# rbrito/deprecated-lame-mirror

Measured on AMD Instinct MI355X. Metric: encoded audio seconds/sec (x real-time) at 44.1kHz stereo CBR128, higher is better.
Workload: dtype f32

## Files before the change

deprecated-lame-mirror_amd/csrc/lh_analysis.hip:

```cpp
#include <stdint.h>
#include <math.h>

#ifdef LH_EMU
#include "hipemu.h"
#define LH_CONST static const
#else
#include <hip/hip_runtime.h>
#define LH_CONST __device__ static const
#endif

#if defined(LH_APROF) && !defined(LH_EMU)
__shared__ unsigned long long *lh_ap_base;
#define LH_PT(var) unsigned long long var = clock64()
#define LH_PA(idx, var) do { if (c.lane == 0) atomicAdd(&lh_ap_base[LH_NPROF * c.wave + 20 + (idx)], clock64() - var); } while (0)
#define LH_PC(idx) do { } while (0)
#endif
#define LH_CUSTOM_LDS "lh_lds_analysis.h"
#define LH_CUSTOM_SMP
#define LH_FZ_X(i) ((((i) >> 4) & 2) | (((i) >> 3) & 24) | (((i) >> 5) & 4))
#define LH_FZ(i) ((i) ^ LH_FZ_X(i))
#define LH_STAGE_IDX(i) LH_FZ(i)
#include "lh_static_tables.h"
#include "lh_dev_common.h"
#if !defined(LH_EMU)
#define LH_KRESTRICT __restrict__
#else
#define LH_KRESTRICT
#endif

#define LH_SPAN (lh_lds.work)
LH_DEVFN float
lh_smp(const LhCtx & c, int ch, int i)
{
    return LH_SPAN[ch * LH_BLKSIZE + LH_FZ(i)];
}

#include "lh_dev_psy_core.h"

struct LhGranuleAt {
    int     live;
    int     gr;
    long long at;
    long long frame_base;
};

LH_DEVFN LhGranuleAt
lh_granule_at(const LhStreamDesc & d, int g)
{
    LhGranuleAt o;
    int const nf = d.frame_end - d.frame_begin;
    int const fr = g / LH_NGR;
    o.live = g < LH_NGR * nf;
    o.gr = g - fr * LH_NGR;
    o.at = d.out_index + d.mid_rel + fr;
    o.frame_base = (long long) (576 * LH_NGR) * (d.frame_begin + fr) - LH_MF_START;
    return o;
}

LH_DEVFN LhStreamDesc
lh_desc_uniform(const LhStreamDesc * descs, int sidx)
{
    LhStreamDesc d = descs[sidx];
    d.pcm_l = lh_uni_ll(d.pcm_l);
    d.pcm_r = lh_uni_ll(d.pcm_r);
    d.pcm_base = lh_uni_ll(d.pcm_base);
    d.nsamples = lh_uni_ll(d.nsamples);
    d.out_index = lh_uni_ll(d.out_index);
    d.mid_rel = lh_uni_i(d.mid_rel);
    d.frame_begin = lh_uni_i(d.frame_begin);
    d.frame_end = lh_uni_i(d.frame_end);
    return d;
}

#ifdef LH_LSF
#define lh_attack_kernel lh_attack_kernel_lsf
#define lh_attack_scan_kernel lh_attack_scan_kernel_lsf
#define lh_analysis_kernel lh_analysis_kernel_lsf
#define lh_launch_analysis lh_launch_analysis_lsf
#define lh_emu_analysis lh_emu_analysis_lsf
#endif

#if defined(LH_APROF) && !defined(LH_EMU)
#define LH_AP_T0() unsigned long long ap_t = clock64()
#define LH_AP(k) do { unsigned long long const n_ = clock64(); if (c.lane == 0) atomicAdd(&aprof[64 * 0 + LH_NPROF * c.wave + (k)], n_ - ap_t); ap_t = n_; } while (0)
#else
#define LH_AP_T0() do { } while (0)
#define LH_AP(k) do { } while (0)
#endif
#define LH_FIR_SPAN 640

#ifndef LH_EMU
extern "C" __global__ void __launch_bounds__(64)
#else
void
#endif
lh_attack_kernel(const LhConfig * LH_KRESTRICT cfg, const int16_t * LH_KRESTRICT pcm, const float *pcmf, const LhStreamDesc * descs, LhMidFrame * frames,
                 int nstreams)
{
    __shared__ float span[2 * LH_FIR_SPAN];
    int const sidx = (int) blockIdx.y;
    LhCtx   c;
    c.cfg = cfg;
    c.T = nullptr;
    c.st = nullptr;
    c.pcm = pcm;
    c.pcmf = pcmf;
    c.d = lh_desc_uniform(descs, sidx);
    c.tid = (int) threadIdx.x;
    c.lane = c.tid;
    c.wave = 0;
    LhGranuleAt const ga = lh_granule_at(c.d, (int) blockIdx.x);
    if (!ga.live)
        return;
    int const lane = c.lane;
    int const n_chn_psy = (cfg->mode == LH_MODE_JOINT_STEREO) ? 4 : cfg->channels;
    int const bufbase = 576 + ga.gr * 576 - LH_FFTOFFSET;
    int const firbase = bufbase + 576 - 350 - LH_NSFIRLEN + 192;
    LhMidGr *mg = &frames[ga.at].small.gr[ga.gr];
    lh_stage_span < LH_FIR_SPAN, 64, 1 > (c, span, span + LH_FIR_SPAN, ga.frame_base + firbase);
    LH_WAVE_SYNC();
    {
        int const i0 = 9 * lane;
        float   x[2][30], y[2][9];
#pragma unroll
        for (int ch = 0; ch < 2; ch++)
#pragma unroll
            for (int t = 0; t < 30; t++)
                x[ch][t] = span[ch * LH_FIR_SPAN + i0 + t];
#pragma unroll
        for (int ch = 0; ch < 2; ch++)
#pragma unroll
            for (int m = 0; m < 9; m++) {
                float   sum1 = x[ch][m + 10], sum2 = 0.0;
#pragma unroll
                for (int j = 0; j < ((LH_NSFIRLEN - 1) / 2) - 1; j += 2) {
                    sum1 += lh_hp_fir[j] * (x[ch][m + j] + x[ch][m + LH_NSFIRLEN - j]);
                    sum2 += lh_hp_fir[j + 1] * (x[ch][m + j + 1] + x[ch][m + LH_NSFIRLEN - j - 1]);
                }
                y[ch][m] = sum1 + sum2;
            }
        LH_WAVE_SYNC();
#pragma unroll
        for (int ch = 0; ch < 2; ch++)
#pragma unroll
            for (int m = 0; m < 9; m++)
                span[ch * LH_FIR_SPAN + i0 + m] = y[ch][m];
    }
    LH_WAVE_SYNC();
    float   fl[9], fr[9];
#pragma unroll
    for (int k = 0; k < 9; k++) {
        fl[k] = span[lane + 64 * k];
        fr[k] = span[LH_FIR_SPAN + lane + 64 * k];
    }
    for (int chn = 0; chn < n_chn_psy; chn++) {
        uint32_t pk[8], pk8 = 0;
#pragma unroll
        for (int k = 0; k < 9; k++) {
            float const l = fl[k], r = fr[k];
            float const v = (chn == 0) ? l : (chn == 1) ? r : (chn == 2) ? l + r : l - r;
            if (k < 8)
                pk[k] = lh_f32_as_u32(lh_fabsf(v));
            else
                pk8 = lh_f32_as_u32(lh_fabsf(v));
        }
        {
            uint32_t const m8 = lh_wave_max8(pk);
            uint32_t const m9 = lh_wave_max_u32(pk8);
            if (lane < 9)
                mg->peak[chn][lane] = lh_u32_as_f32(lane == 8 ? m9 : m8);
        }
    }
}

#ifndef LH_SCAN_BLOCK
#define LH_SCAN_BLOCK 4
#endif
#ifndef LH_EMU
extern "C" __global__ void __launch_bounds__(64)
#else
void
#endif
lh_attack_scan_kernel(const LhConfig * LH_KRESTRICT cfg, const LhTables * LH_KRESTRICT T, const LhStreamDesc * descs, const LhStreamState * states,
                      LhMidFrame * frames, int nstreams)
{
    int const sidx = (int) blockIdx.x;
    int const lane = (int) threadIdx.x;
    LhStreamDesc const d = lh_desc_uniform(descs, sidx);
    int const nf = d.frame_end - d.frame_begin;
    if (nf <= 0)
        return;
    const LhStreamState *st = &states[sidx];
    int const n_chn_psy = lh_uni_i((cfg->mode == LH_MODE_JOINT_STEREO) ? 4 : cfg->channels);
    int const channels = lh_uni_i(cfg->channels), short_blocks = lh_uni_i(cfg->short_blocks);
    int const chn = lane >> 4, i = lane & 15, grp = lane & 48;
    int const mine = chn < n_chn_psy;
    float   le = st->last_en_subshort[chn][i < 9 ? i : 0];
    int     last_att = st->last_attacks[chn];
    float const thresh = T->attack_threshold[chn];
    int     bt_old0 = lh_uni_i(st->blocktype_old[0]), bt_old1 = lh_uni_i(st->blocktype_old[1]);
    int const ng = LH_NGR * nf;
    float   pk_blk[LH_SCAN_BLOCK];
#pragma unroll
    for (int j = 0; j < LH_SCAN_BLOCK; j++) {
        int const g = (j < ng) ? j : 0;
        pk_blk[j] = frames[d.out_index + d.mid_rel + g / LH_NGR].small.gr[g % LH_NGR].peak[chn][i < 9 ? i : 0];
    }
    for (int g0 = 0; g0 < ng; g0 += LH_SCAN_BLOCK) {
        float   pk_cur[LH_SCAN_BLOCK], ssf_blk[LH_SCAN_BLOCK];
        int     nsa_blk[LH_SCAN_BLOCK][4];
#pragma unroll
        for (int j = 0; j < LH_SCAN_BLOCK; j++) {
            int const gn = g0 + LH_SCAN_BLOCK + j, g = (gn < ng) ? gn : 0;
            pk_cur[j] = pk_blk[j];
            pk_blk[j] = frames[d.out_index + d.mid_rel + g / LH_NGR].small.gr[g % LH_NGR].peak[chn][i < 9 ? i : 0];
        }
#pragma unroll
        for (int j = 0; j < LH_SCAN_BLOCK; j++) {
            float const pk = pk_cur[j];
            float const fresh = pk < 1.0f ? 1.0f : pk;
            float const old = lh_shfl_f32(le, grp + ((i + 6) & 15)), older = lh_shfl_f32(le, grp + ((i + 4) & 15));
            float const got = lh_shfl_f32(fresh, grp + ((i - 3) & 15));
            float const e = (i < 3) ? old : got;
            float const e1 = lh_shfl_f32(e, grp + ((i - 1) & 15)), e0 = lh_shfl_f32(e, grp + ((i - 2) & 15));
            float const then = (i < 3) ? older : e0;
            float const ai = (i < 3) ? e / then : (e > then) ? e / then : (then > e * 10.0f) ? then / (e * 10.0f) : 0.0f;
            float const whole = e0 + e1 + e;
            int const tail_low = e * 6 < whole, mid_low = e1 * 6 < whole;
            uint64_t const over_all = lh_ballot(i < 12 && ai > thresh);
            unsigned const over = (unsigned) (over_all >> (16 * chn)) & 0xfffu;
            float   en_short[4];
            en_short[0] = lh_shfl_f32(whole, grp + 2);
            en_short[1] = lh_shfl_f32(whole, grp + 5);
            en_short[2] = lh_shfl_f32(whole, grp + 8);
            en_short[3] = lh_shfl_f32(whole, grp + 11);
            ssf_blk[j] = tail_low ? (mid_low ? 0.25f : 0.5f) : 1.0f;
            int    *nsa = nsa_blk[j];
            le = fresh;
            for (int gq = 0; gq < 4; gq++) {
                unsigned const bits = (over >> (3 * gq)) & 7u;
                nsa[gq] = bits ? ((bits & 1u) ? 1 : (bits & 2u) ? 2 : 3) : 0;
            }
            for (int q = 1; q < 4; q++) {
                float const u = en_short[q - 1];
                float const v = en_short[q];
                float const m = (u > v) ? u : v;
                if (m < 40000) {
                    if (u < 1.7f * v && v < 1.7f * u) {
                        if (q == 1 && nsa[0] <= nsa[q])
                            nsa[0] = 0;
                        nsa[q] = 0;
                    }
                }
            }
        }
#pragma unroll
        for (int j = 0; j < LH_SCAN_BLOCK; j++) {
            int const g = g0 + j;
            if (g >= ng)
                break;
            int const fr = g / LH_NGR, gr = g - fr * LH_NGR;
            LhMidGr *mg = &frames[d.out_index + d.mid_rel + fr].small.gr[gr];
            int    *nsa = nsa_blk[j];
            float const ssf = ssf_blk[j];
            int     uselong = 1;
            if (nsa[0] <= last_att)
                nsa[0] = 0;
            if (last_att == 3 || nsa[0] + nsa[1] + nsa[2] + nsa[3]) {
                uselong = 0;
                if (nsa[1] && nsa[0])
                    nsa[1] = 0;
                if (nsa[2] && nsa[1])
                    nsa[2] = 0;
                if (nsa[3] && nsa[2])
                    nsa[3] = 0;
            }
            if (!mine) {
                nsa[0] = nsa[1] = nsa[2] = nsa[3] = 0;
                uselong = 1;
            }
            else
                last_att = nsa[2];
            if (i == 5 || i == 8 || i == 11)
                mg->sub_short_factor[chn][(i - 5) / 3] = mine ? ssf : 1.0f;
            if (i < 4)
                mg->ns_attacks[chn][i] = (int8_t) (i == 0 ? nsa[0] : i == 1 ? nsa[1] : i == 2 ? nsa[2] : nsa[3]);
            {
                uint64_t const shorts = lh_ballot(!uselong);
                int const s0 = (int) (shorts & 1u), s1 = (int) ((shorts >> 16) & 1u), s23 = (int) ((shorts >> 32) & 0x10001u) != 0;
                int     ul0 = !s0, ul1 = (channels == 2) ? !s1 : 1;
                int     btd[2];
                if (s23)
                    ul0 = ul1 = 0;
                if (short_blocks == 1 && !(ul0 && ul1))
                    ul0 = ul1 = 0;
                if (short_blocks == 2)
                    ul0 = ul1 = 1;
                if (short_blocks == 3)
                    ul0 = ul1 = 0;
                for (int ch = 0; ch < 2; ch++) {
                    int     blocktype = LH_NORM_TYPE;
                    int     was = ch ? bt_old1 : bt_old0;
                    if (ch ? ul1 : ul0) {
                        if (was == LH_SHORT_TYPE)
                            blocktype = LH_STOP_TYPE;
                    }
                    else {
                        blocktype = LH_SHORT_TYPE;
                        if (was == LH_NORM_TYPE)
                            was = LH_START_TYPE;
                        if (was == LH_STOP_TYPE)
                            was = LH_SHORT_TYPE;
                    }
                    btd[ch] = was;
                    if (ch)
                        bt_old1 = lh_uni_i(blocktype);
                    else
                        bt_old0 = lh_uni_i(blocktype);
                }
                if (lane < 2) {
                    mg->uselong[lane] = (int8_t) (lane ? ul1 : ul0);
                    mg->block_type[lane] = (int8_t) (lane ? btd[1] : btd[0]);
                }
            }
        }
    }
}

template < int K1 > LH_DEVFN void
lh_fht_unit_fz(lh_f32x4 tw, float *fz, int u)
{
    constexpr int kx = K1 >> 1, k2 = K1 << 1, k3 = k2 + K1, k4 = k2 << 1;
    int const blk = u / kx, i = u - blk * kx;
    int const axis = (i == 0);
    int const lo = blk * k4 + i;
    int const hi = blk * k4 + (axis ? kx : K1 - i);
    int     al[4], ah[4];
    if (K1 == 4) {
        int const x = LH_FZ_X(lo);
#pragma unroll
        for (int j = 0; j < 4; j++) {
            al[j] = (lo + j * K1) ^ x;
            ah[j] = (hi + j * K1) ^ x;
        }
    }
    else if (K1 == 16) {
        int const x = LH_FZ_X(blk * k4);
#pragma unroll
        for (int j = 0; j < 4; j++) {
            al[j] = (lo + j * K1) ^ x ^ (j >= 2 ? 2 : 0);
            ah[j] = (hi + j * K1) ^ x ^ (j >= 2 ? 2 : 0);
        }
    }
    else if (K1 == 64) {
#pragma unroll
        for (int j = 0; j < 4; j++) {
            al[j] = (lo + j * K1) ^ LH_FZ_X(64 * j);
            ah[j] = (hi + j * K1) ^ (2 ^ LH_FZ_X(64 * j));
        }
    }
    else {
        int const xl = LH_FZ_X(lo), xh = LH_FZ_X(hi);
#pragma unroll
        for (int j = 0; j < 4; j++) {
            al[j] = (lo + j * K1) ^ xl;
            ah[j] = (hi + j * K1) ^ xh;
        }
    }
    float const p0 = fz[al[0]], p1 = fz[al[1]], p2 = fz[al[2]], p3 = fz[al[3]];
    float const q0 = fz[ah[0]], q1 = fz[ah[1]], q2 = fz[ah[2]], q3 = fz[ah[3]];
    float const s01 = p0 + p1, d01 = p0 - p1, s23 = p2 + p3, d23 = p2 - p3;
    float const r2 = (float) (LH_SQRT2 * q2), r3 = (float) (LH_SQRT2 * q3);
    float const t01 = q0 + q1, u01 = q0 - q1;
    float const a_l0 = s01 + s23, a_l1 = d01 + d23, a_l2 = s01 - s23, a_l3 = d01 - d23;
    float const a_h0 = t01 + r2, a_h1 = u01 + r3, a_h2 = t01 - r2, a_h3 = u01 - r3;
    LhRot const rq1 = lh_rot(tw.z, tw.w, p1, q1);
    LhRot const rq3 = lh_rot(tw.z, tw.w, p3, q3);
    float const le = p0 + rq1.along, lm = p0 - rq1.along;
    float const he = q0 + rq1.across, hm = q0 - rq1.across;
    float const l2e = p2 + rq3.along, l2m = p2 - rq3.along;
    float const h2e = q2 + rq3.across, h2m = q2 - rq3.across;
    LhRot const ra = lh_rot(tw.x, tw.y, l2e, h2m);
    LhRot const rb = lh_rot(tw.y, tw.x, h2e, l2m);
    fz[al[0]] = axis ? a_l0 : le + ra.along;
    fz[al[1]] = axis ? a_l1 : lm + rb.across;
    fz[al[2]] = axis ? a_l2 : le - ra.along;
    fz[al[3]] = axis ? a_l3 : lm - rb.across;
    fz[ah[0]] = axis ? a_h0 : he + rb.along;
    fz[ah[1]] = axis ? a_h1 : hm + ra.across;
    fz[ah[2]] = axis ? a_h2 : he - rb.along;
    fz[ah[3]] = axis ? a_h3 : hm - ra.across;
}

LH_DEVFN void
lh_fft_long_inplace(const LhCtx & c, float *x)
{
    const float *w = c.T->fft_window;
    int const lane = c.lane;
    float   o[2][8];
#pragma unroll
    for (int q = 0; q < 2; q++) {
        int const jj = lane + 64 * q;
        int const i = (int) lh_rev8((unsigned) jj);
        const float *xs = x + (i ^ LH_FZ_X(i));
        float   f0, f1, f2, f3, ww;
        f0 = w[i] * xs[0];
        ww = w[i + 0x200] * xs[0x200];
        f1 = f0 - ww;
        f0 = f0 + ww;
        f2 = w[i + 0x100] * xs[0x100];
        ww = w[i + 0x300] * xs[0x300];
        f3 = f2 - ww;
        f2 = f2 + ww;
        o[q][0] = f0 + f2;
        o[q][2] = f0 - f2;
        o[q][1] = f1 + f3;
        o[q][3] = f1 - f3;
        f0 = w[i + 0x001] * xs[0x001];
        ww = w[i + 0x201] * xs[0x201];
        f1 = f0 - ww;
        f0 = f0 + ww;
        f2 = w[i + 0x101] * xs[0x101];
        ww = w[i + 0x301] * xs[0x301];
        f3 = f2 - ww;
        f2 = f2 + ww;
        o[q][4] = f0 + f2;
        o[q][6] = f0 - f2;
        o[q][5] = f1 + f3;
        o[q][7] = f1 - f3;
    }
    {
        lh_f32x4 tw[4][2];
#pragma unroll
        for (int stage = 0; stage < 4; stage++) {
            int const kx = 2 << (2 * stage);
#pragma unroll
            for (int q = 0; q < 2; q++)
                tw[stage][q] = *(const lh_f32x4 *) c.T->fht_tw[stage][(lane + 64 * q) % kx];
        }
        LH_WAVE_SYNC_MEM();
#pragma unroll
        for (int q = 0; q < 2; q++) {
            int const at = 4 * (lane + 64 * q), xa = LH_FZ_X(at);
#pragma unroll
            for (int k = 0; k < 4; k++) {
                x[(at + k) ^ xa] = o[q][k];
                x[(at + k + LH_BLKSIZE / 2) ^ xa] = o[q][4 + k];
            }
        }
        LH_WAVE_SYNC_MEM();
#pragma unroll
        for (int q = 0; q < 2; q++)
            lh_fht_unit_fz < 4 > (tw[0][q], x, lane + 64 * q);
        LH_WAVE_SYNC_MEM();
#pragma unroll
        for (int q = 0; q < 2; q++)
            lh_fht_unit_fz < 16 > (tw[1][q], x, lane + 64 * q);
        LH_WAVE_SYNC_MEM();
#pragma unroll
        for (int q = 0; q < 2; q++)
            lh_fht_unit_fz < 64 > (tw[2][q], x, lane + 64 * q);
        LH_WAVE_SYNC_MEM();
#pragma unroll
        for (int q = 0; q < 2; q++)
            lh_fht_unit_fz < 256 > (tw[3][q], x, lane + 64 * q);
        LH_WAVE_SYNC_MEM();
    }
}

LH_DEVFN void
lh_fft_short_inplace(const LhCtx & c, float *x)
{
    const float *ws = c.T->fft_window_s;
    int const lane = c.lane;
    float   o[2][8];
#pragma unroll
    for (int q = 0; q < 2; q++) {
        int const t = lane + 64 * q, tt = t < 3 * (LH_BLKSIZE_S / 8) ? t : 0;
        int const b = tt >> 5, j = tt & 31;
        int const k = (576 / 3) * (b + 1);
        int const i = (int) lh_rev8((unsigned) (j << 2));
        float   f0, f1, f2, f3, w;
        f0 = ws[i] * x[LH_FZ(i + k)];
        w = ws[0x7f - i] * x[LH_FZ(i + k + 0x80)];
        f1 = f0 - w;
        f0 = f0 + w;
        f2 = ws[i + 0x40] * x[LH_FZ(i + k + 0x40)];
        w = ws[0x3f - i] * x[LH_FZ(i + k + 0xc0)];
        f3 = f2 - w;
        f2 = f2 + w;
        o[q][0] = f0 + f2;
        o[q][2] = f0 - f2;
        o[q][1] = f1 + f3;
        o[q][3] = f1 - f3;
        f0 = ws[i + 0x01] * x[LH_FZ(i + k + 0x01)];
        w = ws[0x7e - i] * x[LH_FZ(i + k + 0x81)];
        f1 = f0 - w;
        f0 = f0 + w;
        f2 = ws[i + 0x41] * x[LH_FZ(i + k + 0x41)];
        w = ws[0x3e - i] * x[LH_FZ(i + k + 0xc1)];
        f3 = f2 - w;
        f2 = f2 + w;
        o[q][4] = f0 + f2;
        o[q][6] = f0 - f2;
        o[q][5] = f1 + f3;
        o[q][7] = f1 - f3;
    }
    LH_WAVE_SYNC_MEM();
#pragma unroll
    for (int q = 0; q < 2; q++) {
        int const t = lane + 64 * q;
        if (t < 3 * (LH_BLKSIZE_S / 8)) {
            int const at = (t >> 5) * LH_BLKSIZE_S + 4 * (t & 31);
#pragma unroll
            for (int k = 0; k < 4; k++) {
                x[LH_FZ(at + k)] = o[q][k];
                x[LH_FZ(at + k + LH_BLKSIZE_S / 2)] = o[q][4 + k];
            }
        }
    }
    LH_WAVE_SYNC_MEM();
    for (int t = lane; t < 3 * (LH_BLKSIZE_S / 8); t += 64) {
        int const b = t >> 5, u = t & 31;
        lh_fht_unit_fz < 4 > (*(const lh_f32x4 *) c.T->fht_tw[0][u % 2], x + b * LH_BLKSIZE_S, u);
    }
    LH_WAVE_SYNC_MEM();
    for (int t = lane; t < 3 * (LH_BLKSIZE_S / 8); t += 64) {
        int const b = t >> 5, u = t & 31;
        lh_fht_unit_fz < 16 > (*(const lh_f32x4 *) c.T->fht_tw[1][u % 8], x + b * LH_BLKSIZE_S, u);
    }
    LH_WAVE_SYNC_MEM();
    for (int t = lane; t < 3 * (LH_BLKSIZE_S / 8); t += 64) {
        int const b = t >> 5, u = t & 31;
        lh_fht_unit_fz < 64 > (*(const lh_f32x4 *) c.T->fht_tw[2][u % 32], x + b * LH_BLKSIZE_S, u);
    }
    LH_WAVE_SYNC_MEM();
}

LH_DEVFN void
lh_an_spectra_short(const LhCtx & c, int w, int both, const float *wl, const float *wr, int first, float *out_own, float *out_ms)
{
    float const sqrt2_half = (float) (LH_SQRT2 * 0.5f);
    int const n = LH_BLKSIZE_S, h = n >> 1;
    for (int m = c.lane; m <= h; m += 64) {
        int const ire = first + m, iim = first + ((m == 0) ? 0 : (n - m));
        float const lre = wl[LH_FZ(ire)], lim = wl[LH_FZ(iim)], rre = wr[LH_FZ(ire)], rim = wr[LH_FZ(iim)];
        float const ore = w ? rre : lre, oim = w ? rim : lim;
        float const mre = (w ? lre - rre : lre + rre) * sqrt2_half, mim = (w ? lim - rim : lim + rim) * sqrt2_half;
        out_own[m] = (m == 0) ? ore * ore : (ore * ore + oim * oim) * 0.5f;
        if (both)
            out_ms[m] = (m == 0) ? mre * mre : (mre * mre + mim * mim) * 0.5f;
    }
}

LH_DEVFN void
lh_an_spectra(const LhCtx & c, int w, int own, int ms, float *work)
{
    float const sqrt2_half = (float) (LH_SQRT2 * 0.5f);
    const float *wl = work, *wr = work + LH_BLKSIZE;
    float   eo[9], em[9];
#pragma unroll
    for (int k = 0; k < 9; k++) {
        int const m0 = c.lane + 64 * k, m = m0 <= LH_BLKSIZE / 2 ? m0 : LH_BLKSIZE / 2;
        int const ire = m, iim = (m == 0) ? 0 : (LH_BLKSIZE - m);
        float const lre = wl[LH_FZ(ire)], lim = wl[LH_FZ(iim)], rre = wr[LH_FZ(ire)], rim = wr[LH_FZ(iim)];
        float const ore = w ? rre : lre, oim = w ? rim : lim;
        float const mre = (w ? lre - rre : lre + rre) * sqrt2_half, mim = (w ? lim - rim : lim + rim) * sqrt2_half;
        eo[k] = (m == 0) ? ore * ore : (ore * ore + oim * oim) * 0.5f;
        em[k] = (m == 0) ? mre * mre : (mre * mre + mim * mim) * 0.5f;
    }
    LH_SYNC_WG_LDS();
#pragma unroll
    for (int k = 0; k < 9; k++) {
        int const m = c.lane + 64 * k;
        if (m <= LH_BLKSIZE / 2) {
            if (own)
                work[w * LH_AN_ROW + m] = eo[k];
            if (ms)
                work[(w + 2) * LH_AN_ROW + m] = em[k];
        }
    }
}

#ifndef LH_EMU
extern "C" __global__ void __launch_bounds__(LH_NT, 6)
#else
void
#endif
lh_analysis_kernel(const LhConfig * LH_KRESTRICT cfg, const LhTables * LH_KRESTRICT T, const int16_t * LH_KRESTRICT pcm, const float *pcmf, const LhStreamDesc * descs,
                   LhMidFrame * frames, int nstreams, LhStreamState * states)
{
#if defined(LH_APROF) && !defined(LH_EMU)
    unsigned long long *aprof = &states[blockIdx.y].prof[0][0];
    if (threadIdx.x == 0)
        lh_ap_base = aprof;
#endif
    LH_AP_T0();
    LhLds & L = lh_lds;
    LhLds & P = L;
    float  *const work = L.work;
#define LH_AN_E(chn) (work + (chn) * LH_AN_ROW)
    int const sidx = (int) blockIdx.y;
    LhCtx   c;
    c.cfg = cfg;
    c.T = T;
    c.st = nullptr;
    c.pcm = pcm;
    c.pcmf = pcmf;
    c.d = lh_desc_uniform(descs, sidx);
    c.tid = (int) threadIdx.x;
    c.lane = c.tid & 63;
    c.wave = lh_uni_i(c.tid >> 6);
    LhGranuleAt const ga = lh_granule_at(c.d, (int) blockIdx.x);
    if (!ga.live)
        return;
    int const lane = c.lane, w = c.wave, gr = ga.gr;
    int const n_chn_psy = (cfg->mode == LH_MODE_JOINT_STEREO) ? 4 : cfg->channels;
    int const bufbase = 576 + gr * 576 - LH_FFTOFFSET;
    LhMidGr *mg = &frames[ga.at].small.gr[gr];
    if (c.tid < 2)
        L.uselong[c.tid] = mg->uselong[c.tid];
    LH_AP(0);
    lh_stage_span < LH_BLKSIZE, LH_NT > (c, LH_SPAN, LH_SPAN + LH_BLKSIZE, ga.frame_base + bufbase);
    LH_SYNC_WG_LDS();
    LH_AP(1);
    if (w < cfg->channels)
        lh_fft_long_inplace(c, work + w * LH_BLKSIZE);
    LH_SYNC_WG_LDS();
    LH_AP(2);
    lh_an_spectra(c, w, w < n_chn_psy, n_chn_psy == 4, work);
    LH_WAVE_SYNC_MEM();
    const float *stg_s3 = T->psy_l.s3;
    LH_WAVE_SYNC_MEM();
    LH_AP(3);
    LH_AP(4);
    {
        int const chn = (lane == 1) ? w + 2 : w;
        int const summing = lane < 3 && chn < n_chn_psy;
        int const loud = (lane == 2);
        float  *prod = (w == 0) ? P.eb : P.thr;
        const float *ew = T->ath_eql_w;
        const float *e = LH_AN_E(summing ? chn : w);
        float   acc = 0.0f;
        for (int h = 0; h < 2; h++) {
            int const j0 = 256 * h;
            LH_WAVE_SYNC_MEM();
#pragma unroll
            for (int q = 0; q < 4; q++) {
                int const j = j0 + lane + 64 * q;
                prod[j - j0] = LH_AN_E(w)[j] * ew[j];
            }
            LH_WAVE_SYNC_MEM();
            if (summing) {
                const lh_f32x4 *s4 = (const lh_f32x4 *) ((loud ? prod - j0 : e) + j0);
                lh_f32x4 a0 = s4[0], a1 = s4[1], a2 = s4[2], a3 = s4[3];
                if (h == 0 && !loud) {
                    a0.x = a0.y = a0.z = a0.w = 0.0f;
                    a1.x = a1.y = a1.z = a1.w = 0.0f;
                    a2.x = a2.y = a2.z = 0.0f;
                }
                for (int g = 0; g < 64; g += 4) {
                    int const n = (g + 4 < 64) ? g + 4 : g;
                    lh_f32x4 const b0 = s4[n], b1 = s4[n + 1], b2 = s4[n + 2], b3 = s4[n + 3];
#ifndef LH_EMU
                    asm volatile("v_add_f32 %0, %0, %1\n\tv_add_f32 %0, %0, %2\n\tv_add_f32 %0, %0, %3\n\tv_add_f32 %0, %0, %4\n\t"
                                 "v_add_f32 %0, %0, %5\n\tv_add_f32 %0, %0, %6\n\tv_add_f32 %0, %0, %7\n\tv_add_f32 %0, %0, %8\n\t"
                                 "v_add_f32 %0, %0, %9\n\tv_add_f32 %0, %0, %10\n\tv_add_f32 %0, %0, %11\n\tv_add_f32 %0, %0, %12\n\t"
                                 "v_add_f32 %0, %0, %13\n\tv_add_f32 %0, %0, %14\n\tv_add_f32 %0, %0, %15\n\tv_add_f32 %0, %0, %16"
                                 : "+v"(acc)
                                 : "v"(a0.x), "v"(a0.y), "v"(a0.z), "v"(a0.w), "v"(a1.x), "v"(a1.y), "v"(a1.z), "v"(a1.w),
                                   "v"(a2.x), "v"(a2.y), "v"(a2.z), "v"(a2.w), "v"(a3.x), "v"(a3.y), "v"(a3.z), "v"(a3.w));
#else
                    acc += a0.x; acc += a0.y; acc += a0.z; acc += a0.w;
                    acc += a1.x; acc += a1.y; acc += a1.z; acc += a1.w;
                    acc += a2.x; acc += a2.y; acc += a2.z; acc += a2.w;
                    acc += a3.x; acc += a3.y; acc += a3.z; acc += a3.w;
#endif
                    a0 = b0;
                    a1 = b1;
                    a2 = b2;
                    a3 = b3;
                }
            }
        }
        if (summing) {
            if (!loud) {
                acc += e[LH_BLKSIZE / 2];
                mg->tot_ener[chn] = acc;
            }
            else {
                acc = (float) (acc * LH_VO_SCALE);
                mg->loud[w] = acc;
            }
        }
        LH_WAVE_SYNC_MEM();
    }
    LH_SYNC_WG_LDS();
    LH_AP(5);
    {
        LhMidLong *ml = &frames[ga.at].lng;
        if (n_chn_psy == 4) {
            LhMaskChan const two[2] = {
                {w, LH_AN_E(w), &P.eb[w * 64], &P.thr[w * 64], nullptr, nullptr, &ml->m[gr][w]},
                {w + 2, LH_AN_E(w + 2), &P.eb[(w + 2) * 64], &P.thr[(w + 2) * 64], nullptr, nullptr, &ml->m[gr][w + 2]}
            };
            lh_compute_masking < 2, 1 > (c, 1, two, stg_s3);
        }
        else if (w < n_chn_psy) {
            LhMaskChan const one[1] = { {w, LH_AN_E(w), &P.eb[w * 64], &P.thr[w * 64], nullptr, nullptr, &ml->m[gr][w]} };
            lh_compute_masking < 1, 1 > (c, 1, one, stg_s3);
        }
    }
    LH_AP(6);
    int const any_short = lh_uni_i(!(L.uselong[0] && L.uselong[1]));
    if (!any_short)
        return;
    LH_SYNC_WG_LDS();
    lh_stage_span < LH_BLKSIZE, LH_NT > (c, LH_SPAN, LH_SPAN + LH_BLKSIZE, ga.frame_base + bufbase);
    LH_SYNC_WG_LDS();
    if (!L.uselong[w])
        lh_fft_short_inplace(c, work + w * LH_BLKSIZE);
    LH_SYNC_WG_LDS();
    for (int sblock = 0; sblock < 3; sblock++) {
        if (w < n_chn_psy && !L.uselong[w]) {
            LhMidShort *ms = &frames[ga.at].shrt;
            int const both = (n_chn_psy == 4);
            lh_an_spectra_short(c, w, both, work, work + LH_BLKSIZE, sblock * LH_BLKSIZE_S, L.eshort[w], L.eshort[w + 2 < 4 ? w + 2 : 3]);
            LH_WAVE_SYNC_MEM();
            if (both) {
                LhMaskChan const two[2] = {
                    {w, L.eshort[w], &P.eb[w * 64], &P.thr[w * 64], nullptr, nullptr, &ms->m[gr][sblock][w]},
                    {w + 2, L.eshort[w + 2], &P.eb[(w + 2) * 64], &P.thr[(w + 2) * 64], nullptr, nullptr, &ms->m[gr][sblock][w + 2]}
                };
                lh_compute_masking < 2, 1 > (c, 0, two, T->psy_s.s3);
            }
            else {
                LhMaskChan const one[1] = { {w, L.eshort[w], &P.eb[w * 64], &P.thr[w * 64], nullptr, nullptr, &ms->m[gr][sblock][w]} };
                lh_compute_masking < 1, 1 > (c, 0, one, T->psy_s.s3);
            }
        }
        LH_SYNC_WG_LDS();
    }
    LH_AP(7);
}

#ifndef LH_EMU
extern "C" int
lh_launch_analysis(const LhConfig * cfg, const LhTables * T, const int16_t * pcm, const float *pcmf, const LhStreamDesc * descs,
                   const LhStreamState * states, LhMidPools mid, int nstreams, int max_frames, void *stream)
{
    if (nstreams <= 0 || max_frames <= 0)
        return 0;
    dim3 const grid((unsigned) (LH_NGR * max_frames), (unsigned) nstreams);
    hipLaunchKernelGGL(lh_attack_kernel, grid, dim3(64), 0, (hipStream_t) stream, cfg, pcm, pcmf, descs, mid.frames, nstreams);
    hipLaunchKernelGGL(lh_attack_scan_kernel, dim3((unsigned) nstreams), dim3(64), 0, (hipStream_t) stream, cfg, T, descs, states,
                       mid.frames, nstreams);
    hipLaunchKernelGGL(lh_analysis_kernel, grid, dim3(LH_NT), 0, (hipStream_t) stream, cfg, T, pcm, pcmf, descs, mid.frames, nstreams,
                       (LhStreamState *) states);
    return (int) hipGetLastError();
}
#else
extern "C" int
lh_emu_analysis(const LhConfig * cfg, const LhTables * T, const int16_t * pcm, const float *pcmf, const LhStreamDesc * descs,
                const LhStreamState * states, const LhMidPools * pools, int nstreams, int max_frames)
{
    LhMidPools const mid = *pools;
    hipemu_dim3 grid = { (unsigned) (LH_NGR * max_frames), (unsigned) nstreams, 1 }, b64 = { 64, 1, 1 }, b128 = { LH_NT, 1, 1 };
    hipemu_dim3 grid1 = { (unsigned) nstreams, 1, 1 };
    hipemu_run(grid, b64,[=] () {
               lh_attack_kernel(cfg, pcm, pcmf, descs, mid.frames, nstreams);
               }
    );
    hipemu_run(grid1, b64,[=] () {
               lh_attack_scan_kernel(cfg, T, descs, states, mid.frames, nstreams);
               }
    );
    hipemu_run(grid, b128,[=] () {
               lh_analysis_kernel(cfg, T, pcm, pcmf, descs, mid.frames, nstreams, (LhStreamState *) states);
               }
    );
    return 0;
}
#endif
```

deprecated-lame-mirror_amd/csrc/lh_dev_common.h:

```cpp
#ifndef LH_DEV_COMMON_H
#define LH_DEV_COMMON_H

#include <stdint.h>
#include "lamehip_types.h"
#include "lh_device.h"
#include "lh_wave.h"
#include "lh_dev_math.h"

#define LH_NT 128
#ifdef LH_LSF
#define LH_NGR 1
#define LH_IS_LSF 1
#define LH_RATE8K(c) ((c).rate8k)
#else
#define LH_NGR 2
#define LH_IS_LSF 0
#define LH_RATE8K(c) 0
#endif
#define LH_BLOCK LH_NT
#define LH_SQRT2 1.41421356237309504880

#ifdef LH_EMU
#define LH_SYNC_WG() do { __syncthreads(); } while (0)
#define LH_SYNC_WG_LDS() do { __syncthreads(); } while (0)
// ... 445 lines not shown
    const int16_t *pcm;
    const float *pcmf;
    LhStreamDesc d;
    long long frame_base;
    int     lane, wave, tid;
    int     ns, ns_amp, sfb21_extra, full_outer_loop, subblock_gain;
    int     rate8k;
    int     l21;
};

LH_DEVFN void
lh_ctx_hot(LhCtx & c)
{
    c.ns = lh_uni_i(c.cfg->noise_shaping);
    c.ns_amp = lh_uni_i(c.cfg->noise_shaping_amp);
    c.sfb21_extra = lh_uni_i(c.cfg->sfb21_extra);
    c.full_outer_loop = lh_uni_i(c.cfg->full_outer_loop);
    c.subblock_gain = lh_uni_i(c.cfg->subblock_gain);
    c.l21 = lh_uni_i(c.T->sfb_l[LH_SBPSY_L]);
#ifdef LH_LSF
    c.rate8k = lh_uni_i(c.cfg->samplerate <= 8000);
#else
    c.rate8k = 0;
#endif
}

#ifdef LH_DEBUG_DUMP
#define LH_ROUTE(c, k) do { if ((c).lane == 0) (c).st->dbg_route[(c).wave][k] += 1u; } while (0)
#else
#define LH_ROUTE(c, k) do { } while (0)
#endif
#define LH_ROUTE_ZERO(bt) ((bt) == LH_NORM_TYPE ? LH_RT_ZERO_norm : (bt) == LH_SHORT_TYPE ? LH_RT_ZERO_short : LH_RT_ZERO_other)

#ifdef LH_EMU
#define LH_AS_GLOBAL(type, p) (p)
#else
template < typename X > __device__ __forceinline__ X *
lh_as_global(X * p)
{
    typedef __attribute__((address_space(1))) X GX;
    unsigned long long const u = (unsigned long long) p;
    unsigned lo = (unsigned) __builtin_amdgcn_readfirstlane((int) (unsigned) u);
    unsigned hi = (unsigned) __builtin_amdgcn_readfirstlane((int) (unsigned) (u >> 32));
    asm volatile("" : "+s"(lo), "+s"(hi));
    return (X *) (GX *) (((unsigned long long) hi << 32) | lo);
}
#define LH_AS_GLOBAL(type, p) lh_as_global < type > (p)
#endif
LH_DEVFN LhCtx
lh_ctx_load(void)
{
    LhCtx   o;
    o.cfg = LH_AS_GLOBAL(const LhConfig, lh_lds.ctx.cfg);
    o.T = LH_AS_GLOBAL(const LhTables, lh_lds.ctx.T);
    o.st = LH_AS_GLOBAL(LhStreamState, lh_lds.ctx.st);
    o.pcm = LH_AS_GLOBAL(const int16_t, lh_lds.ctx.pcm);
    o.pcmf = LH_AS_GLOBAL(const float, lh_lds.ctx.pcmf);
    o.d = lh_lds.ctx.d;
    o.frame_base = lh_lds.ctx.frame_base;
    o.tid = (int) threadIdx.x;
    o.lane = o.tid & 63;
    o.wave = lh_uni_i(o.tid >> 6);
    lh_ctx_hot(o);
    return o;
}

LH_DEVFN int
lh_cfg_class(const LhCtx & c)
{
    int const ok = !LH_IS_LSF && (c.ns == 1 || c.ns == 2) && c.ns_amp == 1 && c.full_outer_loop == 0 && c.sfb21_extra == 0
        && c.l21 <= 418;
    return ok ? c.ns : 0;
}

LH_DEVFN int
lh_granule_is_usual(const LhCtx & c, int block_type, int substep)
{
    return (block_type == LH_NORM_TYPE && (substep & 2) == 0) ? lh_cfg_class(c) : 0;
}

LH_DEVFN int
lh_granule_is_usual_short(const LhCtx & c, int block_type, int substep)
{
    return (block_type == LH_SHORT_TYPE && (substep & 2) == 0 && c.subblock_gain == 1) ? lh_cfg_class(c) : 0;
}

LH_DEVFN void
lh_pin_usual(LhCtx & c, int nsh)
{
    if (nsh)
        c.ns = nsh;
    c.ns_amp = 1;
    c.full_outer_loop = 0;
    c.sfb21_extra = 0;
    c.rate8k = 0;
    if (c.l21 > 418)
        __builtin_unreachable();
}

LH_DEVFN void
lh_pin_usual(LhQR & R)
{
    R.block_type = LH_NORM_TYPE;
    R.sfb_lmax = LH_SBPSY_L;
    R.sfb_smin = LH_SBPSY_S;
    R.psy_lmax = LH_SBPSY_L;
    R.psymax = LH_SBPSY_L;
    R.sfbmax = LH_SBPSY_L;
    R.sfbdivide = 11;
    if ((R.substep_shaping & 2) != 0)
        __builtin_unreachable();
}

LH_DEVFN void
lh_pin_usual_short(LhQR & R)
{
    R.block_type = LH_SHORT_TYPE;
    R.sfb_lmax = 0;
    R.sfb_smin = 0;
    R.psy_lmax = 0;
    R.psymax = 3 * LH_SBPSY_S;
    R.sfbmax = 3 * LH_SBPSY_S;
    R.sfbdivide = 3 * LH_SBPSY_S - 18;
    if ((R.substep_shaping & 2) != 0)
        __builtin_unreachable();
}

LH_DEVFN void
lh_rg_put(const LhCtx & c, const LhQR & R, const LhGrR & g)
{
    if (c.lane == 0) {
        lh_lds.rg[c.wave].R = R;
        lh_lds.rg[c.wave].g = g;
    }
    LH_WAVE_SYNC();
}

LH_DEVFN void
lh_stage_window(const LhCtx & c, float (*mf)[LH_MF_NEEDED], long long base)
{
    float const scale = c.cfg->pcm_scale;
    long long const last = c.d.nsamples - 1;
    float const mix = c.cfg->pcm_mix;
    float const scale_r = c.cfg->pcm_scale_r;
    if (c.pcmf) {
        for (int t = c.tid; t < 2 * LH_MF_NEEDED; t += LH_NT) {
            int const ch = t >= LH_MF_NEEDED, i = t - ch * LH_MF_NEEDED;
            long long const p = base + i;
            float   v = 0.0f;
            if (p >= 0 && p <= last && p >= c.d.pcm_base)
                v = c.pcmf[(ch == 0 ? c.d.pcm_l : c.d.pcm_r) + (p - c.d.pcm_base)];
            mf[ch][i] = v;
        }
        return;
    }
    if (mix != 0.0f) {
        for (int i = c.tid; i < LH_MF_NEEDED; i += LH_NT) {
            long long const p = base + i;
            float   v = 0.0f;
            if (p >= 0 && p <= last && p >= c.d.pcm_base) {
                float const xl = (float) c.pcm[c.d.pcm_l + (p - c.d.pcm_base)];
                float const xr = (float) c.pcm[c.d.pcm_r + (p - c.d.pcm_base)];
                v = xl * scale + xr * mix;
            }
            mf[0][i] = v;
            mf[1][i] = 0.0f;
        }
        return;
    }
    {
        long long const lo = base, hi = base + LH_MF_NEEDED - 1;
        long long const ol = c.d.pcm_l + (base - c.d.pcm_base), orr = c.d.pcm_r + (base - c.d.pcm_base);
        int const inside = lo >= 0 && lo >= c.d.pcm_base && hi <= last && ((ol | orr) & 1) == 0;
        if (lh_uni_i(inside)) {
            const uint32_t *pl = (const uint32_t *) (c.pcm + ol), *pr = (const uint32_t *) (c.pcm + orr);
            uint32_t v[16];
#pragma unroll
            for (int u = 0; u < 8; u++) {
                int const j = c.tid + LH_NT * u;
                int const jj = j < LH_MF_NEEDED / 2 ? j : LH_MF_NEEDED / 2 - 1;
                v[u] = pl[jj];
                v[8 + u] = pr[jj];
            }
#pragma unroll
            for (int u = 0; u < 8; u++) {
                int const j = c.tid + LH_NT * u;
                if (j < LH_MF_NEEDED / 2) {
                    lh_f32x2 a, b;
                    a.x = (float) (int16_t) (v[u] & 0xffffu) * scale;
                    a.y = (float) (int16_t) (v[u] >> 16) * scale;
                    b.x = (float) (int16_t) (v[8 + u] & 0xffffu) * scale_r;
                    b.y = (float) (int16_t) (v[8 + u] >> 16) * scale_r;
                    ((lh_f32x2 *) mf[0])[j] = a;
                    ((lh_f32x2 *) mf[1])[j] = b;
                }
            }
            return;
        }
    }
    for (int t0 = c.tid; t0 < 2 * LH_MF_NEEDED; t0 += 6 * LH_NT) {
        int16_t v[6];
#pragma unroll
        for (int u = 0; u < 6; u++) {
            int const t = t0 + u * LH_NT;
            int const tt = t < 2 * LH_MF_NEEDED ? t : 2 * LH_MF_NEEDED - 1;
            int const ch = tt >= LH_MF_NEEDED, i = tt - ch * LH_MF_NEEDED;
            long long p = base + i;
            p = p < 0 ? 0 : (p > last ? last : p);
            p = p < c.d.pcm_base ? c.d.pcm_base : p;
            v[u] = (c.d.nsamples > 0) ? c.pcm[(ch == 0 ? c.d.pcm_l : c.d.pcm_r) + (p - c.d.pcm_base)] : (int16_t) 0;
        }
#pragma unroll
        for (int u = 0; u < 6; u++) {
            int const t = t0 + u * LH_NT;
            if (t < 2 * LH_MF_NEEDED) {
                int const ch = t >= LH_MF_NEEDED, i = t - ch * LH_MF_NEEDED;
                long long const p = base + i;
                mf[ch][i] = (p < 0 || p > last) ? 0.0f : (float) v[u] * (ch == 0 ? scale : scale_r);
            }
        }
    }
}

#ifndef LH_STAGE_IDX
#define LH_STAGE_IDX(i) (i)
#endif
template < int N, int NT, int PLAIN = 0 > LH_DEVFN void
lh_stage_span(const LhCtx & c, float *d0, float *d1, long long base)
{
#define LH_STAGE_AT(i) (PLAIN ? (i) : LH_STAGE_IDX(i))
    float const scale = c.cfg->pcm_scale;
    long long const last = c.d.nsamples - 1;
    float const mix = c.cfg->pcm_mix;
    float const scale_r = c.cfg->pcm_scale_r;
    if (c.pcmf) {
        for (int t = c.tid; t < 2 * N; t += NT) {
            int const ch = t >= N, i = t - ch * N;
            long long const p = base + i;
            float   v = 0.0f;
            if (p >= 0 && p <= last && p >= c.d.pcm_base)
                v = c.pcmf[(ch == 0 ? c.d.pcm_l : c.d.pcm_r) + (p - c.d.pcm_base)];
            (ch ? d1 : d0)[LH_STAGE_AT(i)] = v;
        }
        return;
    }
    if (mix != 0.0f) {
        for (int i = c.tid; i < N; i += NT) {
            long long const p = base + i;
            float   v = 0.0f;
            if (p >= 0 && p <= last && p >= c.d.pcm_base) {
                float const xl = (float) c.pcm[c.d.pcm_l + (p - c.d.pcm_base)];
                float const xr = (float) c.pcm[c.d.pcm_r + (p - c.d.pcm_base)];
                v = xl * scale + xr * mix;
            }
            d0[LH_STAGE_AT(i)] = v;
            d1[LH_STAGE_AT(i)] = 0.0f;
        }
        return;
    }
    {
        long long const lo = base, hi = base + N - 1;
        long long const ol = c.d.pcm_l + (base - c.d.pcm_base), orr = c.d.pcm_r + (base - c.d.pcm_base);
        int const inside = lo >= 0 && lo >= c.d.pcm_base && hi <= last && ((ol | orr) & 1) == 0;
        static_assert(N % 2 == 0, "pairs");
        constexpr int U = (N / 2 + NT - 1) / NT;
        if (lh_uni_i(inside)) {
            const uint32_t *pl = (const uint32_t *) (c.pcm + ol), *pr = (const uint32_t *) (c.pcm + orr);
            uint32_t v[2 * U];
#pragma unroll
            for (int u = 0; u < U; u++) {
                int const j = c.tid + NT * u;
                int const jj = j < N / 2 ? j : N / 2 - 1;
                v[u] = pl[jj];
                v[U + u] = pr[jj];
            }
#pragma unroll
            for (int u = 0; u < U; u++) {
                int const j = c.tid + NT * u;
                if (j < N / 2) {
                    lh_f32x2 a, b;
                    a.x = (float) (int16_t) (v[u] & 0xffffu) * scale;
                    a.y = (float) (int16_t) (v[u] >> 16) * scale;
                    b.x = (float) (int16_t) (v[U + u] & 0xffffu) * scale_r;
                    b.y = (float) (int16_t) (v[U + u] >> 16) * scale_r;
                    *(lh_f32x2 *) &d0[LH_STAGE_AT(2 * j)] = a;
                    *(lh_f32x2 *) &d1[LH_STAGE_AT(2 * j)] = b;
                }
            }
            return;
        }
    }
    for (int t = c.tid; t < 2 * N; t += NT) {
        int const ch = t >= N, i = t - ch * N;
        long long const p0 = base + i;
        long long p = p0 < 0 ? 0 : (p0 > last ? last : p0);
        int16_t v;
        p = p < c.d.pcm_base ? c.d.pcm_base : p;
        v = (c.d.nsamples > 0) ? c.pcm[(ch == 0 ? c.d.pcm_l : c.d.pcm_r) + (p - c.d.pcm_base)] : (int16_t) 0;
        (ch ? d1 : d0)[LH_STAGE_AT(i)] = (p0 < 0 || p0 > last) ? 0.0f : (float) v * (ch == 0 ? scale : scale_r);
    }
}
#undef LH_STAGE_AT

#ifndef LH_CUSTOM_SMP
LH_DEVFN float
lh_smp(const LhCtx & c, int ch, int i)
{
    return lh_lds.mf[ch][i];
}
#endif

#endif
```

Before: 84340.

## Batch attack-kernel granules per block and prefetch next span into registers

After: 84110. About the same (-0.3%).

```diff
diff --git a/deprecated-lame-mirror_amd/csrc/lh_analysis.hip b/deprecated-lame-mirror_amd/csrc/lh_analysis.hip
--- a/deprecated-lame-mirror_amd/csrc/lh_analysis.hip
+++ b/deprecated-lame-mirror_amd/csrc/lh_analysis.hip
@@ -88,6 +88,9 @@
 #define LH_AP(k) do { } while (0)
 #endif
 #define LH_FIR_SPAN 640
+#ifndef LH_ATK_RUN
+#define LH_ATK_RUN 8
+#endif
 
 #ifndef LH_EMU
 extern "C" __global__ void __launch_bounds__(64)
@@ -109,68 +112,84 @@
     c.tid = (int) threadIdx.x;
     c.lane = c.tid;
     c.wave = 0;
-    LhGranuleAt const ga = lh_granule_at(c.d, (int) blockIdx.x);
-    if (!ga.live)
-        return;
     int const lane = c.lane;
     int const n_chn_psy = (cfg->mode == LH_MODE_JOINT_STEREO) ? 4 : cfg->channels;
-    int const bufbase = 576 + ga.gr * 576 - LH_FFTOFFSET;
-    int const firbase = bufbase + 576 - 350 - LH_NSFIRLEN + 192;
-    LhMidGr *mg = &frames[ga.at].small.gr[ga.gr];
-    lh_stage_span < LH_FIR_SPAN, 64, 1 > (c, span, span + LH_FIR_SPAN, ga.frame_base + firbase);
-    LH_WAVE_SYNC();
-    {
-        int const i0 = 9 * lane;
-        float   x[2][30], y[2][9];
-#pragma unroll
-        for (int ch = 0; ch < 2; ch++)
-#pragma unroll
-            for (int t = 0; t < 30; t++)
-                x[ch][t] = span[ch * LH_FIR_SPAN + i0 + t];
-#pragma unroll
-        for (int ch = 0; ch < 2; ch++)
-#pragma unroll
-            for (int m = 0; m < 9; m++) {
-                float   sum1 = x[ch][m + 10], sum2 = 0.0;
-#pragma unroll
-                for (int j = 0; j < ((LH_NSFIRLEN - 1) / 2) - 1; j += 2) {
-                    sum1 += lh_hp_fir[j] * (x[ch][m + j] + x[ch][m + LH_NSFIRLEN - j]);
-                    sum2 += lh_hp_fir[j + 1] * (x[ch][m + j + 1] + x[ch][m + LH_NSFIRLEN - j - 1]);
+    int const ng = LH_NGR * (c.d.frame_end - c.d.frame_begin);
+    int const g0 = LH_ATK_RUN * (int) blockIdx.x;
+    int const g1 = (g0 + LH_ATK_RUN < ng) ? g0 + LH_ATK_RUN : ng;
+    if (g0 >= g1)
+        return;
+#define LH_ATK_BASE(ga) ((ga).frame_base + (576 + (ga).gr * 576 - LH_FFTOFFSET) + 576 - 350 - LH_NSFIRLEN + 192)
+    LhGranuleAt ga = lh_granule_at(c.d, g0);
+    LhSpanRegs < LH_FIR_SPAN > nl = lh_span_load < LH_FIR_SPAN > (c, 0, LH_ATK_BASE(ga));
+    LhSpanRegs < LH_FIR_SPAN > nr = lh_span_load < LH_FIR_SPAN > (c, 1, LH_ATK_BASE(ga));
+    for (int g = g0; g < g1; g++) {
+        LhMidGr *mg = &frames[ga.at].small.gr[ga.gr];
+        c.lane = (int) lh_vec_u32((uint32_t) lane);
+        lh_span_store < LH_FIR_SPAN, 1 > (c, nl, 0, span);
+        lh_span_store < LH_FIR_SPAN, 1 > (c, nr, 1, span + LH_FIR_SPAN);
+        if (g + 1 < g1) {
+            ga = lh_granule_at(c.d, g + 1);
+            nl = lh_span_load < LH_FIR_SPAN > (c, 0, LH_ATK_BASE(ga));
+            nr = lh_span_load < LH_FIR_SPAN > (c, 1, LH_ATK_BASE(ga));
+        }
+        LH_WAVE_SYNC();
+        {
+            int const i0 = 9 * lane;
+            float   x[2][30], y[2][9];
+#pragma unroll
+            for (int ch = 0; ch < 2; ch++)
+#pragma unroll
+                for (int t = 0; t < 30; t++)
+                    x[ch][t] = span[ch * LH_FIR_SPAN + i0 + t];
+#pragma unroll
+            for (int ch = 0; ch < 2; ch++)
+#pragma unroll
+                for (int m = 0; m < 9; m++) {
+                    float   sum1 = x[ch][m + 10], sum2 = 0.0;
+#pragma unroll
+                    for (int j = 0; j < ((LH_NSFIRLEN - 1) / 2) - 1; j += 2) {
+                        sum1 += lh_hp_fir[j] * (x[ch][m + j] + x[ch][m + LH_NSFIRLEN - j]);
+                        sum2 += lh_hp_fir[j + 1] * (x[ch][m + j + 1] + x[ch][m + LH_NSFIRLEN - j - 1]);
+                    }
+                    y[ch][m] = sum1 + sum2;
                 }
-                y[ch][m] = sum1 + sum2;
-            }
+            LH_WAVE_SYNC();
+#pragma unroll
+            for (int ch = 0; ch < 2; ch++)
+#pragma unroll
+                for (int m = 0; m < 9; m++)
+                    span[ch * LH_FIR_SPAN + i0 + m] = y[ch][m];
+        }
         LH_WAVE_SYNC();
-#pragma unroll
-        for (int ch = 0; ch < 2; ch++)
-#pragma unroll
-            for (int m = 0; m < 9; m++)
-                span[ch * LH_FIR_SPAN + i0 + m] = y[ch][m];
-    }
-    LH_WAVE_SYNC();
-    float   fl[9], fr[9];
-#pragma unroll
-    for (int k = 0; k < 9; k++) {
-        fl[k] = span[lane + 64 * k];
-        fr[k] = span[LH_FIR_SPAN + lane + 64 * k];
-    }
-    for (int chn = 0; chn < n_chn_psy; chn++) {
-        uint32_t pk[8], pk8 = 0;
+        float   fl[9], fr[9];
 #pragma unroll
         for (int k = 0; k < 9; k++) {
-            float const l = fl[k], r = fr[k];
-            float const v = (chn == 0) ? l : (chn == 1) ? r : (chn == 2) ? l + r : l - r;
-            if (k < 8)
-                pk[k] = lh_f32_as_u32(lh_fabsf(v));
-            else
-                pk8 = lh_f32_as_u32(lh_fabsf(v));
-        }
-        {
-            uint32_t const m8 = lh_wave_max8(pk);
-            uint32_t const m9 = lh_wave_max_u32(pk8);
-            if (lane < 9)
-                mg->peak[chn][lane] = lh_u32_as_f32(lane == 8 ? m9 : m8);
-        }
-    }
+            fl[k] = span[lane + 64 * k];
+            fr[k] = span[LH_FIR_SPAN + lane + 64 * k];
+        }
+        for (int chn = 0; chn < n_chn_psy; chn++) {
+            uint32_t pk[8], pk8 = 0;
+#pragma unroll
+            for (int k = 0; k < 9; k++) {
+                float const l = fl[k], r = fr[k];
+                float const v = (chn == 0) ? l : (chn == 1) ? r : (chn == 2) ? l + r : l - r;
+                if (k < 8)
+                    pk[k] = lh_f32_as_u32(lh_fabsf(v));
+                else
+                    pk8 = lh_f32_as_u32(lh_fabsf(v));
+            }
+            {
+                uint32_t const m8 = lh_wave_max8(pk);
+                uint32_t const m9 = lh_wave_max_u32(pk8);
+                if (lane < 9)
+                    mg->peak[chn][lane] = lh_u32_as_f32(lane == 8 ? m9 : m8);
+            }
+        }
+
+        LH_WAVE_SYNC();
+    }
+#undef LH_ATK_BASE
 }
 
 #ifndef LH_SCAN_BLOCK
@@ -752,7 +771,8 @@
     if (nstreams <= 0 || max_frames <= 0)
         return 0;
     dim3 const grid((unsigned) (LH_NGR * max_frames), (unsigned) nstreams);
-    hipLaunchKernelGGL(lh_attack_kernel, grid, dim3(64), 0, (hipStream_t) stream, cfg, pcm, pcmf, descs, mid.frames, nstreams);
+    dim3 const runs((unsigned) ((LH_NGR * max_frames + LH_ATK_RUN - 1) / LH_ATK_RUN), (unsigned) nstreams);
+    hipLaunchKernelGGL(lh_attack_kernel, runs, dim3(64), 0, (hipStream_t) stream, cfg, pcm, pcmf, descs, mid.frames, nstreams);
     hipLaunchKernelGGL(lh_attack_scan_kernel, dim3((unsigned) nstreams), dim3(64), 0, (hipStream_t) stream, cfg, T, descs, states,
                        mid.frames, nstreams);
     hipLaunchKernelGGL(lh_analysis_kernel, grid, dim3(LH_NT), 0, (hipStream_t) stream, cfg, T, pcm, pcmf, descs, mid.frames, nstreams,
@@ -767,7 +787,8 @@
     LhMidPools const mid = *pools;
     hipemu_dim3 grid = { (unsigned) (LH_NGR * max_frames), (unsigned) nstreams, 1 }, b64 = { 64, 1, 1 }, b128 = { LH_NT, 1, 1 };
     hipemu_dim3 grid1 = { (unsigned) nstreams, 1, 1 };
-    hipemu_run(grid, b64,[=] () {
+    hipemu_dim3 runs = { (unsigned) ((LH_NGR * max_frames + LH_ATK_RUN - 1) / LH_ATK_RUN), (unsigned) nstreams, 1 };
+    hipemu_run(runs, b64,[=] () {
                lh_attack_kernel(cfg, pcm, pcmf, descs, mid.frames, nstreams);
                }
     );
diff --git a/deprecated-lame-mirror_amd/csrc/lh_dev_common.h b/deprecated-lame-mirror_amd/csrc/lh_dev_common.h
--- a/deprecated-lame-mirror_amd/csrc/lh_dev_common.h
+++ b/deprecated-lame-mirror_amd/csrc/lh_dev_common.h
@@ -771,6 +771,123 @@
 }
 #undef LH_STAGE_AT
 
+enum { LH_SPAN_MIXED = 0, LH_SPAN_PAIRS = 1, LH_SPAN_S16 = 2, LH_SPAN_F32 = 3 };
+template < int N > struct LhSpanRegs {
+    static_assert(N % 2 == 0 && N < (1 << 19), "pairs; positions relative to the span fit LH_SPAN_FAR");
+    static constexpr int U = (N / 2 + 63) / 64;
+    uint32_t v[2 * U];
+    int     kind;
+    int     lo0, lop, hi;
+    long long base;
+};
+
+#define LH_SPAN_FAR (1 << 20)
+LH_DEVFN int
+lh_span_rel(long long x)
+{
+    return (int) (x < -LH_SPAN_FAR ? -LH_SPAN_FAR : (x > LH_SPAN_FAR ? LH_SPAN_FAR : x));
+}
+
+template < int N > LH_DEVFN LhSpanRegs < N >
+lh_span_load(const LhCtx & c, int ch, long long base)
+{
+    constexpr int U = LhSpanRegs < N >::U;
+    LhSpanRegs < N > r;
+    long long const last = c.d.nsamples - 1;
+    long long const plane = (ch == 0) ? c.d.pcm_l : c.d.pcm_r;
+    long long const first = c.d.pcm_base > 0 ? c.d.pcm_base : 0;
+    r.base = base;
+    r.lo0 = lh_span_rel(-base);
+    r.lop = lh_span_rel(first - base);
+    r.hi = lh_span_rel(last - base);
+#pragma unroll
+    for (int u = 0; u < 2 * U; u++)
+        r.v[u] = 0;
+    if (c.pcmf == nullptr && c.cfg->pcm_mix != 0.0f) {
+        r.kind = LH_SPAN_MIXED;
+        return r;
+    }
+    if (c.pcmf == nullptr) {
+        long long const o = plane + (base - c.d.pcm_base);
+        int const inside = base >= 0 && base >= c.d.pcm_base && base + N - 1 <= last && (o & 1) == 0;
+        if (lh_uni_i(inside)) {
+            const uint32_t *pp = (const uint32_t *) (c.pcm + o);
+            r.kind = LH_SPAN_PAIRS;
+#pragma unroll
+            for (int u = 0; u < U; u++) {
+                int const j = c.lane + 64 * u;
+                r.v[u] = pp[j < N / 2 ? j : N / 2 - 1];
+            }
+            return r;
+        }
+    }
+    r.kind = c.pcmf ? LH_SPAN_F32 : LH_SPAN_S16;
+    if (c.d.nsamples > 0) {
+        long long const anchor = (base > last ? last : base) < first ? first : (base > last ? last : base);
+        long long const o = plane + (anchor - c.d.pcm_base);
+        int const a0 = (0 < r.hi ? 0 : r.hi) < r.lop ? r.lop : (0 < r.hi ? 0 : r.hi);
+#pragma unroll
+        for (int u = 0; u < 2 * U; u++) {
+            int const i = c.lane + 64 * u < N ? c.lane + 64 * u : N - 1;
+            int const m = i < r.hi ? i : r.hi;
+            int const rel = (m < r.lop ? r.lop : m) - a0;
+            r.v[u] = c.pcmf ? lh_f32_as_u32((c.pcmf + o)[rel]) : (uint32_t) (uint16_t) (c.pcm + o)[rel];
+        }
+    }
+    return r;
+}
+
+template < int N, int PLAIN = 0 > LH_DEVFN void
+lh_span_store(const LhCtx & c, const LhSpanRegs < N > &r, int ch, float *d)
+{
+#define LH_STAGE_AT(i) (PLAIN ? (i) : LH_STAGE_IDX(i))
+    constexpr int U = LhSpanRegs < N >::U;
+    float const scale = (ch == 0) ? c.cfg->pcm_scale : c.cfg->pcm_scale_r;
+    if (r.kind == LH_SPAN_PAIRS) {
+#pragma unroll
+        for (int u = 0; u < U; u++) {
+            int const j = c.lane + 64 * u;
+            if (j < N / 2) {
+                lh_f32x2 a;
+                a.x = (float) (int16_t) (r.v[u] & 0xffffu) * scale;
+                a.y = (float) (int16_t) (r.v[u] >> 16) * scale;
+                *(lh_f32x2 *) & d[LH_STAGE_AT(2 * j)] = a;
+            }
+        }
+    }
+    else if (r.kind == LH_SPAN_S16) {
+#pragma unroll
+        for (int u = 0; u < 2 * U; u++) {
+            int const i = c.lane + 64 * u;
+            if (i < N)
+                d[LH_STAGE_AT(i)] = (i < r.lo0 || i > r.hi) ? 0.0f : (float) (int16_t) r.v[u] * scale;
+        }
+    }
+    else if (r.kind == LH_SPAN_F32) {
+#pragma unroll
+        for (int u = 0; u < 2 * U; u++) {
+            int const i = c.lane + 64 * u;
+            if (i < N)
+                d[LH_STAGE_AT(i)] = (i >= r.lop && i <= r.hi) ? lh_u32_as_f32(r.v[u]) : 0.0f;
+        }
+    }
+    else {
+        long long const last = c.d.nsamples - 1;
+        float const mix = c.cfg->pcm_mix;
+        for (int i = c.lane; i < N; i += 64) {
+            long long const p = r.base + i;
+            float   v = 0.0f;
+            if (ch == 0 && p >= 0 && p <= last && p >= c.d.pcm_base) {
+                float const xl = (float) c.pcm[c.d.pcm_l + (p - c.d.pcm_base)];
+                float const xr = (float) c.pcm[c.d.pcm_r + (p - c.d.pcm_base)];
+                v = xl * c.cfg->pcm_scale + xr * mix;
+            }
+            d[LH_STAGE_AT(i)] = v;
+        }
+    }
+#undef LH_STAGE_AT
+}
+
 #ifndef LH_CUSTOM_SMP
 LH_DEVFN float
 lh_smp(const LhCtx & c, int ch, int i)
```
